# jinli99/iShapEditing

Measured on AMD Instinct MI355X. Metric: end-to-end drag-edit wall-clock (s) per shape, lower is better.
Workload: dtype f16; 1 GPU; C3 chair drag-edit: 3 handle->target pairs, 40 guided iterations (UNet fwd + drag gradient + UNet input-grad bwd + DDPM update) + 256^3 occupancy decode; unet=421M params, 1x96x128x128 latent, fp16 torso, r1=12, scale=1200

## Files before the change

### include/ishap.h

```cpp
#ifndef ISHAP_H
#define ISHAP_H
#ifdef __cplusplus
extern "C" {
#endif

const char* ishap_last_error(void);
int ishap_device_status(void);
int ishap_rendezvous_would_grant(const void* owner, void* stream);
int ishap_version(void);

typedef struct ishap_unet ishap_unet;

typedef struct {
  int image_size;
  int in_channels;
  int model_channels;
  int out_channels;
  int num_res_blocks;
  int n_mult;
  int channel_mult[8];
  int n_att;
  int attention_ds[8];
  int num_head_channels;
  int max_batch;
} ishap_unet_config;

int ishap_unet_create(const ishap_unet_config* cfg, int device, ishap_unet** out);
void ishap_unet_destroy(ishap_unet* u);

int ishap_unet_num_params(const ishap_unet* u);
int ishap_unet_param_info(const ishap_unet* u, int index, char* name, int name_cap, int* ndim, long long* shape);
int ishap_unet_load_param(ishap_unet* u, const char* name, const float* data, long long numel, void* stream);
int ishap_unet_params_loaded(const ishap_unet* u);

int ishap_unet_forward(ishap_unet* u, const float* x, const float* timesteps, int N, int feat_layer,
                       float* out, void* inter_feat, int keep_for_backward, void* stream);
int ishap_unet_tap_shape(const ishap_unet* u, int feat_layer, int* channels, int* size);
const void* ishap_unet_tap_ptr(const ishap_unet* u);
int ishap_unet_join_tail(ishap_unet* u, void* stream);
int ishap_unet_run_tail(ishap_unet* u);
int ishap_unet_marks(ishap_unet* u, int* tags, float* ms, int cap, float* tail_begin_ms, float* tail_end_ms);
int ishap_unet_copy_tap(const ishap_unet* u, void* dst, void* stream);
int ishap_unet_block_output(const ishap_unet* u, int group, int index, int* channels, int* size, void* dst_nchw_f16,
                            void* stream);
int ishap_unet_prepare_timesteps(ishap_unet* u, const float* timesteps, int n, void* stream);
long long ishap_unet_workspace_bytes(const ishap_unet* u);

int ishap_unet_snapshot_save(ishap_unet* u, void* stream);
int ishap_unet_snapshot_restore(ishap_unet* u, void* stream);
int ishap_unet_snapshot_drop(ishap_unet* u);
long long ishap_unet_snapshot_bytes(const ishap_unet* u);

int ishap_unet_backward_input(ishap_unet* u, const void* cot_nhwc, const float* scale2, float* dx, void* stream);
int ishap_unet_backward_from_output(ishap_unet* u, const void* cot_out, int cot_is_f16, const float* scale2, float* dx,
                                    void* stream);

long long ishap_group_norm32_scratch_bytes(int N, int HW, int C);
int ishap_group_norm32(const void* x_nhwc_f16, const float* gamma, const float* beta, int N, int H, int W, int C, int silu,
                       int route, void* y_nhwc_f16, float* stats, void* scratch, void* stream);
int ishap_group_norm32_backward(const void* g_nhwc_f16, const void* x_nhwc_f16, const float* stats, const float* gamma,
                                const float* beta, int N, int H, int W, int C, int silu, int route, void* dx_nhwc_f16,
                                void* scratch, void* stream);
int ishap_group_norm32_plan(int N, int H, int W, int C, int backward, int pending, int film, int act, int pool, int gmode, int route,
                            int* route_out, int* parts, int* vec, int* threads, int* grid_x, int* grid_y, int* lds_bytes,
                            int* xcd, char* kernel, int kernel_cap);

typedef struct {
  int backward, N, H, W, C, route, film, act;
  int pool, split;
  int gmode, sums_ready;
  int csplit, emb_ld;
  const float *gamma, *beta, *emb;
  void* scratch;
  const void *x, *x2;
  void *xcopy, *out, *xpool;
  float* stats_out;
  const long long *sums, *sums2;
  const void* g;
  const float* stats;
  const void *add, *add2;
  void *dx, *dx2;
  long long* csums;
  const float* ws;
  int nslab, ldr, res_ups, reserved_;
  long long zstride;
  const float *bias, *bias2;
  const void* res;
  void* ya;
} ishap_group_norm_desc;
int ishap_group_norm32_run(const ishap_group_norm_desc* d, int launch, void* stream, int* route_out, int* parts_out, char* kernel,
                           int kernel_cap);

typedef struct {
  float min_log;
  float max_log;
  float sqrt_recip;
  float sqrt_recipm1;
  float coef1, coef2;
  float nonzero;
  int clip_denoised;
  int mode;
  float ddim_a;
  float ddim_b;
  float ddim_sigma;
  int rng;
  unsigned long long rng_seed, rng_offset;
  float* noise_out;
} ishap_step_coefs;
int ishap_ddpm_step(const float* x, const float* model_out, const float* noise, const float* variance_in,
                    const ishap_step_coefs* k, int N, int C, int HW,
                    float* sample, float* pred_xstart, float* variance, float* mean, void* stream);
int ishap_ddpm_step_guided(const float* x, const float* model_out, const float* noise, const float* variance_in,
                           const ishap_step_coefs* k, int N, int C, int HW, const float* grad, float scale,
                           const float* grad_mul_dev, float* guided, float* sample, float* variance, void* stream);
int ishap_ddpm_step_guided_scales(const float* x, const float* model_out, const float* noise, const float* variance_in,
                                  const ishap_step_coefs* k, int N, int C, int HW, const float* grad, const float* scales,
                                  const float* grad_mul_dev, float* guided, float* sample, float* variance, void* stream);
int ishap_guided_update(const float* sample, const float* variance, const float* grad, float scale,
                        const float* grad_mul_dev, long long numel, float* out, void* stream);
int ishap_axpby(const float* x, const float* y, float a, float b, long long numel, float* out, void* stream);

typedef struct {
  int W;
  int ld;
  int Cc;
  const int* chmap;
  const float* sources;
  const float* targets;
// ... 194 lines not shown
```

### ishapediting_amd/_lib.py

```python
from __future__ import annotations

import ctypes as C
import os

HERE = os.path.dirname(os.path.abspath(__file__))
LIB_PATH = os.path.join(HERE, "libishap_hip.so")

c_float_p = C.POINTER(C.c_float)
c_void_p = C.c_void_p


class UNetConfigC(C.Structure):
    _fields_ = [("image_size", C.c_int), ("in_channels", C.c_int), ("model_channels", C.c_int),
                ("out_channels", C.c_int), ("num_res_blocks", C.c_int), ("n_mult", C.c_int),
                ("channel_mult", C.c_int * 8), ("n_att", C.c_int), ("attention_ds", C.c_int * 8),
                ("num_head_channels", C.c_int), ("max_batch", C.c_int)]


class StepCoefs(C.Structure):
    _fields_ = [("min_log", C.c_float), ("max_log", C.c_float), ("sqrt_recip", C.c_float),
                ("sqrt_recipm1", C.c_float), ("coef1", C.c_float), ("coef2", C.c_float),
                ("nonzero", C.c_float), ("clip_denoised", C.c_int), ("mode", C.c_int),
                ("ddim_a", C.c_float), ("ddim_b", C.c_float), ("ddim_sigma", C.c_float),
                ("rng", C.c_int), ("rng_seed", C.c_ulonglong), ("rng_offset", C.c_ulonglong), ("noise_out", c_void_p)]
# ... 9 lines not shown
    _fields_ = [("E", C.c_int), ("W", C.c_int), ("ld", C.c_int), ("Cc", C.c_int), ("chmap", c_void_p), ("sources", c_void_p),
                ("targets", c_void_p), ("handle_offsets", C.POINTER(C.c_int)), ("r", C.c_int), ("voxel", C.c_float),
                ("cof", C.POINTER(C.c_float)), ("l1", C.c_int), ("orig_stride", C.c_longlong), ("scratch", c_void_p),
                ("scratch_bytes", C.c_longlong)]


class IgemmBufC(C.Structure):
    _fields_ = [("ptr", c_void_p), ("bytes", C.c_longlong)]


class IgemmDescC(C.Structure):
    _fields_ = ([(f, C.c_int) for f in ("M", "N", "Cin", "taps", "K2", "H", "W", "ldx", "ldx2", "ldw", "ldo", "ldr", "ups",
                                        "res_ups", "out_mode", "pending", "chunk_tiles")] +
                [(f, IgemmBufC) for f in ("X", "X2", "Wt", "out", "bias", "bias2", "res", "ws", "stat_out", "gb_x", "gb_stats",
                                          "gb_gamma", "gb_beta", "gb_emb", "gb_csums")] +
                [("gb_emb_ld", C.c_int), ("gb_film", C.c_int), ("gb_act", C.c_int)])


class AttnDescC(C.Structure):
    _fields_ = ([(f, C.c_int) for f in ("pass_", "N", "T", "C", "heads", "d", "xcd_map")] +
                [(f, IgemmBufC) for f in ("qkv", "out", "lse", "dout", "dqkv")])


class Attn8DescC(C.Structure):
    _fields_ = ([(f, C.c_int) for f in ("N", "C", "heads")] +
                [(f, IgemmBufC) for f in ("xn", "wqkv", "bqkv", "wproj", "qkv", "aout", "lse", "slices", "flags")])


class GroupNormDescC(C.Structure):
    _fields_ = ([(f, C.c_int) for f in ("backward", "N", "H", "W", "C", "route", "film", "act", "pool", "split", "gmode",
                                        "sums_ready", "csplit", "emb_ld")] +
                [(f, c_void_p) for f in ("gamma", "beta", "emb", "scratch", "x", "x2", "xcopy", "out", "xpool", "stats_out", "sums",
                                         "sums2", "g", "stats", "add", "add2", "dx", "dx2", "csums", "ws")] +
                [(f, C.c_int) for f in ("nslab", "ldr", "res_ups", "reserved_")] + [("zstride", C.c_longlong)] +
                [(f, c_void_p) for f in ("bias", "bias2", "res", "ya")])


class DecoderWeightsC(C.Structure):
    _fields_ = [("B", c_void_p), ("W1", c_void_p), ("b1", c_void_p), ("W2", c_void_p), ("b2", c_void_p),
                ("w3", c_void_p), ("b3", c_void_p)]


class CameraC(C.Structure):
    _fields_ = [("eye", C.c_float * 3), ("centre", C.c_float * 3), ("up", C.c_float * 3), ("fov_y_deg", C.c_float),
                ("near", C.c_float), ("far", C.c_float)]


SYMBOLS = {
    "ishap_last_error": (C.c_char_p, []),
    "ishap_version": (C.c_int, []),
    "ishap_device_status": (C.c_int, []),
    "ishap_rendezvous_would_grant": (C.c_int, [C.c_void_p, C.c_void_p]),
    "ishap_group_norm32_scratch_bytes": (C.c_longlong, [C.c_int, C.c_int, C.c_int]),
    "ishap_group_norm32": (C.c_int, [c_void_p, c_void_p, c_void_p, C.c_int, C.c_int, C.c_int, C.c_int, C.c_int, C.c_int,
                                     c_void_p, c_void_p, c_void_p, c_void_p]),
    "ishap_group_norm32_backward": (C.c_int, [c_void_p, c_void_p, c_void_p, c_void_p, c_void_p, C.c_int, C.c_int, C.c_int,
                                              C.c_int, C.c_int, C.c_int, c_void_p, c_void_p, c_void_p]),
    "ishap_group_norm32_plan": (C.c_int, [C.c_int] * 11 + [C.POINTER(C.c_int)] * 8 + [C.c_char_p, C.c_int]),
    "ishap_group_norm32_run": (C.c_int, [C.POINTER(GroupNormDescC), C.c_int, c_void_p, C.POINTER(C.c_int), C.POINTER(C.c_int),
                                         C.c_char_p, C.c_int]),
    "ishap_unet_create": (C.c_int, [C.POINTER(UNetConfigC), C.c_int, C.POINTER(c_void_p)]),
    "ishap_unet_destroy": (None, [c_void_p]),
    "ishap_unet_num_params": (C.c_int, [c_void_p]),
    "ishap_unet_param_info": (C.c_int, [c_void_p, C.c_int, C.c_char_p, C.c_int, C.POINTER(C.c_int),
                                        C.POINTER(C.c_longlong)]),
    "ishap_unet_load_param": (C.c_int, [c_void_p, C.c_char_p, c_void_p, C.c_longlong, c_void_p]),
    "ishap_unet_params_loaded": (C.c_int, [c_void_p]),
    "ishap_unet_forward": (C.c_int, [c_void_p, c_void_p, c_float_p, C.c_int, C.c_int, c_void_p, c_void_p, C.c_int,
                                     c_void_p]),
    "ishap_unet_tap_shape": (C.c_int, [c_void_p, C.c_int, C.POINTER(C.c_int), C.POINTER(C.c_int)]),
    "ishap_unet_tap_ptr": (c_void_p, [c_void_p]),
    "ishap_unet_copy_tap": (C.c_int, [c_void_p, c_void_p, c_void_p]),
    "ishap_unet_block_output": (C.c_int, [c_void_p, C.c_int, C.c_int, C.POINTER(C.c_int), C.POINTER(C.c_int), c_void_p,
                                          c_void_p]),
    "ishap_unet_workspace_bytes": (C.c_longlong, [c_void_p]),
    "ishap_unet_join_tail": (C.c_int, [c_void_p, c_void_p]),
    "ishap_unet_run_tail": (C.c_int, [c_void_p]),
    "ishap_unet_snapshot_save": (C.c_int, [c_void_p, c_void_p]),
    "ishap_unet_snapshot_restore": (C.c_int, [c_void_p, c_void_p]),
    "ishap_unet_snapshot_drop": (C.c_int, [c_void_p]),
    "ishap_unet_snapshot_bytes": (C.c_longlong, [c_void_p]),
    "ishap_unet_marks": (C.c_int, [c_void_p, c_void_p, c_void_p, C.c_int, c_void_p, c_void_p]),
    "ishap_unet_prepare_timesteps": (C.c_int, [c_void_p, c_void_p, C.c_int, c_void_p]),
    "ishap_unet_backward_input": (C.c_int, [c_void_p, c_void_p, c_void_p, c_void_p, c_void_p]),
    "ishap_unet_backward_from_output": (C.c_int, [c_void_p, c_void_p, C.c_int, c_void_p, c_void_p, c_void_p]),
    "ishap_triplane_points_loss_grad": (C.c_int, [c_void_p, C.c_int, C.POINTER(DecoderWeightsC), c_void_p, c_void_p, c_void_p,
                                                  c_void_p, C.c_longlong, c_void_p, c_void_p, c_void_p, c_void_p]),
    "ishap_x0_grad_to_cotangent": (C.c_int, [c_void_p, c_void_p, c_void_p, c_void_p, C.c_float, C.c_float, C.c_int, C.c_int,
                                             c_void_p, c_void_p, c_void_p]),
    "ishap_ddpm_step": (C.c_int, [c_void_p, c_void_p, c_void_p, c_void_p, C.POINTER(StepCoefs), C.c_int, C.c_int,
                                  C.c_int, c_void_p, c_void_p, c_void_p, c_void_p, c_void_p]),
    "ishap_ddpm_step_guided": (C.c_int, [c_void_p, c_void_p, c_void_p, c_void_p, C.POINTER(StepCoefs), C.c_int, C.c_int, C.c_int,
                                         c_void_p, C.c_float, c_void_p, c_void_p, c_void_p, c_void_p, c_void_p]),
    "ishap_ddpm_step_guided_scales": (C.c_int, [c_void_p, c_void_p, c_void_p, c_void_p, C.POINTER(StepCoefs), C.c_int, C.c_int,
                                                C.c_int, c_void_p, c_void_p, c_void_p, c_void_p, c_void_p, c_void_p, c_void_p]),
    "ishap_guided_update": (C.c_int, [c_void_p, c_void_p, c_void_p, C.c_float, c_void_p, C.c_longlong, c_void_p,
                                      c_void_p]),
    "ishap_axpby": (C.c_int, [c_void_p, c_void_p, C.c_float, C.c_float, C.c_longlong, c_void_p, c_void_p]),
    "ishap_drag_setup": (C.c_int, [C.POINTER(DragArgsC), c_void_p]),
    "ishap_drag_loss_grad": (C.c_int, [C.POINTER(DragArgsC), c_void_p, c_void_p, c_void_p, c_void_p, c_void_p]),
    "ishap_drag_loss_cotangent": (C.c_int, [C.POINTER(DragArgsC), c_void_p, c_void_p, c_void_p, c_void_p, c_void_p, c_void_p,
                                            c_void_p, c_void_p]),
    "ishap_drag_batch_scratch_bytes": (C.c_longlong, [C.c_int, C.c_int, C.c_int]),
    "ishap_drag_batch_setup": (C.c_int, [C.POINTER(DragBatchArgsC), c_void_p]),
    "ishap_drag_batch_loss_grad": (C.c_int, [C.POINTER(DragBatchArgsC), c_void_p, c_void_p, c_void_p, c_void_p, c_void_p]),
    "ishap_drag_batch_loss_cotangent": (C.c_int, [C.POINTER(DragBatchArgsC), c_void_p, c_void_p, c_void_p, c_void_p, c_void_p,
                                                  c_void_p, c_void_p, c_void_p]),
    "ishap_grad_to_scaled_f16": (C.c_int, [c_void_p, c_void_p, c_void_p, c_void_p, C.c_longlong, c_void_p]),
    "ishap_planes_prepare": (C.c_int, [c_void_p, c_void_p, c_void_p, C.c_int, c_void_p, c_void_p]),
    "ishap_triplane_fit_loss_grad": (C.c_int, [c_void_p, C.c_int, C.POINTER(DecoderWeightsC), c_void_p, c_void_p, c_void_p,
                                               C.c_longlong, c_void_p, c_void_p, C.c_longlong, C.c_float, c_void_p, c_void_p,
                                               c_void_p]),
    "ishap_triplane_reg_adam_step": (C.c_int, [c_void_p, c_void_p, c_void_p, c_void_p, c_void_p, C.c_int, c_void_p, C.c_double,
                                               C.c_double, C.c_double, C.c_double, C.c_float, C.c_float, c_void_p, c_void_p,
                                               c_void_p]),
    "ishap_triplane_reg_values": (C.c_int, [c_void_p, C.c_int, c_void_p, c_void_p, c_void_p]),
    "ishap_triplane_decode_points": (C.c_int, [c_void_p, C.c_int, C.POINTER(DecoderWeightsC), c_void_p, C.c_longlong,
                                               c_void_p, c_void_p]),
    "ishap_surface_scratch_bytes": (C.c_longlong, [C.c_int]),
    "ishap_surface_count": (C.c_int, [c_void_p, C.c_int, C.c_float, C.c_int, c_void_p, c_void_p, c_void_p]),
    "ishap_surface_emit": (C.c_int, [c_void_p, C.c_int, C.c_float, C.c_int, c_void_p, c_void_p, c_void_p, c_void_p]),
    "ishap_mesh_smooth_scratch_bytes": (C.c_longlong, [C.c_longlong, C.c_longlong]),
    "ishap_mesh_smooth": (C.c_int, [c_void_p, C.c_longlong, c_void_p, C.c_longlong, C.c_int, C.c_float, c_void_p, C.c_longlong, c_void_p]),
    "ishap_chamfer": (C.c_int, [c_void_p, C.c_longlong, c_void_p, C.c_longlong, c_void_p, c_void_p, c_void_p]),
    "ishap_mesh_tri_areas": (C.c_int, [c_void_p, c_void_p, C.c_longlong, c_void_p, c_void_p]),
    "ishap_mesh_points_on_tris": (C.c_int, [c_void_p, c_void_p, c_void_p, c_void_p, C.c_longlong, c_void_p, c_void_p]),
    "ishap_mesh_occupancy": (C.c_int, [c_void_p, c_void_p, C.c_longlong, c_void_p, C.c_longlong, c_void_p, c_void_p]),
    "ishap_mesh_distance_scratch_bytes": (C.c_longlong, [C.c_longlong]),
    "ishap_mesh_distance": (C.c_int, [c_void_p, c_void_p, C.c_longlong, c_void_p, C.c_longlong, C.c_int, c_void_p, c_void_p,
                                      c_void_p, C.c_longlong, c_void_p]),
    "ishap_mesh_distance_scratch_bytes_sdf": (C.c_longlong, [C.c_longlong, C.c_longlong, C.c_int]),
    "ishap_hausdorff": (C.c_int, [c_void_p, C.c_longlong, c_void_p, C.c_longlong, c_void_p, c_void_p, c_void_p]),
    "ishap_winding_scratch_bytes": (C.c_longlong, [C.c_longlong, C.c_longlong]),
    "ishap_mesh_winding": (C.c_int, [c_void_p, c_void_p, C.c_longlong, c_void_p, C.c_longlong, c_void_p, c_void_p, C.c_longlong,
                                     c_void_p]),
    "ishap_cloud_winding": (C.c_int, [c_void_p, c_void_p, c_void_p, C.c_longlong, c_void_p, C.c_longlong, c_void_p, c_void_p,
                                      C.c_longlong, c_void_p]),
    "ishap_cloud_areas": (C.c_int, [c_void_p, C.c_longlong, C.c_int, c_void_p, c_void_p]),
    "ishap_cloud_knn": (C.c_int, [c_void_p, C.c_longlong, C.c_int, c_void_p, c_void_p, c_void_p]),
    "ishap_cloud_normals": (C.c_int, [c_void_p, C.c_longlong, c_void_p, C.c_int, c_void_p, c_void_p, c_void_p]),
    "ishap_cloud_orient_scratch_bytes": (C.c_longlong, [C.c_longlong]),
    "ishap_cloud_orient": (C.c_int, [c_void_p, c_void_p, c_void_p, C.c_longlong, C.c_int, c_void_p, C.c_longlong,
                                     C.POINTER(C.c_int), c_void_p]),
    "ishap_volume_label": (C.c_int, [c_void_p, C.c_int, C.c_int, C.c_int, C.c_float, C.c_int, C.c_int, c_void_p, c_void_p]),
    "ishap_volume_components_scratch_bytes": (C.c_longlong, [C.c_longlong]),
    "ishap_volume_components_count": (C.c_int, [c_void_p, C.c_int, C.c_int, C.c_int, c_void_p, c_void_p, c_void_p]),
    "ishap_volume_components_emit": (C.c_int, [c_void_p, C.c_int, C.c_int, C.c_int, c_void_p, c_void_p, c_void_p]),
    "ishap_volume_flip": (C.c_int, [c_void_p, c_void_p, c_void_p, C.c_int, C.c_int, C.c_int, C.c_float, c_void_p, C.c_longlong,
                                    c_void_p, c_void_p]),
    "ishap_group_field_stats": (C.c_int, [c_void_p, c_void_p, C.c_int, C.c_longlong, C.c_int, c_void_p, c_void_p]),
    "ishap_arap_scratch_bytes": (C.c_longlong, [C.c_longlong, C.c_longlong, C.c_longlong]),
    "ishap_arap": (C.c_int, [c_void_p, C.c_longlong, c_void_p, C.c_longlong, c_void_p, c_void_p, C.c_longlong, C.c_int, C.c_double,
                             C.c_longlong, c_void_p, c_void_p, c_void_p, c_void_p, C.c_longlong, c_void_p]),
    "ishap_nearest_vertices": (C.c_int, [c_void_p, C.c_longlong, c_void_p, C.c_longlong, c_void_p, c_void_p]),
    "ishap_render_scratch_bytes": (C.c_longlong, [C.c_longlong, C.c_longlong, C.c_int, C.c_int]),
    "ishap_render_mesh": (C.c_int, [c_void_p, C.c_longlong, c_void_p, C.c_longlong, c_void_p, c_void_p, c_void_p, C.c_int,
                                    C.POINTER(CameraC), C.c_int, C.c_int, c_void_p, C.c_longlong, c_void_p, c_void_p, c_void_p,
                                    c_void_p]),
    "ishap_unproject": (C.c_int, [C.POINTER(CameraC), C.c_int, C.c_int, c_void_p, C.c_longlong, c_void_p, c_void_p]),
    "ishap_profile_begin": (C.c_int, []),
    "ishap_profile_end": (C.c_int, [C.POINTER(C.c_double), C.c_int]),
    "ishap_profile_shapes": (C.c_int, [C.c_char_p, C.c_int]),
    "ishap_igemm_plan": (C.c_int, [C.c_int] * 10 + [C.POINTER(C.c_int), C.POINTER(C.c_int), C.c_char_p, C.c_int]),
    "ishap_igemm_run": (C.c_int, [C.POINTER(IgemmDescC), C.c_int, c_void_p, C.POINTER(C.c_int), C.c_char_p, C.c_int]),
    "ishap_igemm_reduce": (C.c_int, [C.POINTER(IgemmDescC), C.c_int, C.c_int, c_void_p]),
    "ishap_attention_run": (C.c_int, [C.POINTER(AttnDescC), C.c_int, c_void_p, C.c_char_p, C.c_int]),
    "ishap_attention8_run": (C.c_int, [C.POINTER(Attn8DescC), C.c_int, C.c_int, c_void_p, C.POINTER(C.c_int)]),
    "ishap_triplane_decode_grid": (C.c_int, [c_void_p, C.c_int, C.POINTER(DecoderWeightsC), c_void_p, C.c_int,
                                             c_void_p, c_void_p]),
}

_lib = None


def lib():
    global _lib
    if _lib is None:
        if not os.path.exists(LIB_PATH):
            raise RuntimeError(
                f"{LIB_PATH} is missing: the HIP extension is required (no CPU fallback exists). "
                "Build it with `python -m ishapediting_amd.build`.")
        import torch
        tlib = os.path.join(os.path.dirname(torch.__file__), "lib", "libamdhip64.so")
        if os.path.exists(tlib):
            C.CDLL(tlib, mode=C.RTLD_GLOBAL)
        l = C.CDLL(LIB_PATH)
        for name, (res, args) in SYMBOLS.items():
            fn = getattr(l, name)
            fn.restype = res
            fn.argtypes = args
        if l.ishap_version() < 16:
            raise RuntimeError(f"{LIB_PATH} is an older build (ABI {l.ishap_version()} < 16): rebuild with `python -m ishapediting_amd.build`")
        _lib = l
    return _lib


def check(rc: int):
    if rc != 0:
        msg = lib().ishap_last_error()
        raise RuntimeError(f"libishap_hip: {msg.decode() if msg else 'error'} (code {rc})")


def ptr(t):
    return None if t is None else t.data_ptr()


def stream_ptr(device=None):
    import torch
    return torch.cuda.current_stream(device).cuda_stream
```

### ishapediting_amd/csrc/misc.hip

```cpp
#include "misc.h"

__global__ __launch_bounds__(256) void nchw_to_nhwc_kernel(const float* __restrict__ src, half_t* __restrict__ dst,
                                                           int C, int HW, int Cpad, int ytiles, uint4* __restrict__ zero, long long zero_n16) {
  __shared__ float tile[32][33];
  const int n = blockIdx.z;
  if ((int)blockIdx.y >= ytiles) {
    const long long nb = (long long)gridDim.x * (gridDim.y - ytiles) * gridDim.z;
    const long long b = blockIdx.x + (long long)gridDim.x * ((blockIdx.y - ytiles) + (long long)(gridDim.y - ytiles) * blockIdx.z);
    for (long long i = b * 256 + threadIdx.x; i < zero_n16; i += nb * 256) zero[i] = make_uint4(0u, 0u, 0u, 0u);
    return;
  }
  const int p0 = blockIdx.x * 32, c0 = blockIdx.y * 32;
  const int tx = threadIdx.x & 31, ty = threadIdx.x >> 5;
  for (int j = ty; j < 32; j += 8) {
    int c = c0 + j, p = p0 + tx;
    tile[j][tx] = (c < C && p < HW) ? src[((long long)n * C + c) * HW + p] : 0.f;
  }
  __syncthreads();
  for (int j = ty; j < 32; j += 8) {
    int p = p0 + j, c = c0 + tx;
    if (p < HW && c < Cpad) dst[((long long)n * HW + p) * Cpad + c] = (half_t)tile[tx][j];
  }
}
int nchw_f32_to_nhwc_f16(const float* src, half_t* dst, int N, int C, int HW, int Cpad, hipStream_t s, void* zero, size_t zero_bytes) {
// ... 43 lines not shown
  const int tx = threadIdx.x & 31, ty = threadIdx.x >> 5;
  for (int j = ty; j < 32; j += 8) {
    int c = c0 + j, p = p0 + tx;
    tile[j][tx] = (c < C && p < HW) ? (float)src[((long long)n * C + c) * HW + p] * mul : 0.f;
  }
  __syncthreads();
  for (int j = ty; j < 32; j += 8) {
    int p = p0 + j, c = c0 + tx;
    if (p < HW && c < ld) dst[((long long)n * HW + p) * ld + c] = (half_t)tile[tx][j];
  }
}
int nchw_to_nhwc_f16_scaled(const void* src, int src_f32, half_t* dst, int N, int C, int HW, int ld, float mul,
                            hipStream_t s) {
  dim3 g(ceil_div(HW, 32), ceil_div(ld, 32), N);
  if (src_f32) hipLaunchKernelGGL(nchw_any_to_nhwc_kernel<float>, g, dim3(256), 0, s, (const float*)src, dst, C, HW, ld, mul);
  else hipLaunchKernelGGL(nchw_any_to_nhwc_kernel<half_t>, g, dim3(256), 0, s, (const half_t*)src, dst, C, HW, ld, mul);
  ISHAP_CHECK_HIP(hipGetLastError());
  return 0;
}

__global__ void concat2_kernel(const half_t* __restrict__ a, const half_t* __restrict__ b, half_t* __restrict__ o,
                               long long M, int Ca, int Cb, const long long* __restrict__ sa,
                               const long long* __restrict__ sb, long long* __restrict__ so, int N) {
  if (so && blockIdx.x == 0) {
    const int Cc = Ca + Cb;
    for (int i = threadIdx.x; i < N * Cc * 2; i += blockDim.x) {
      const int k = i & 1, c = (i >> 1) % Cc, n = (i >> 1) / Cc;
      so[i] = c < Ca ? sa[(n * Ca + c) * 2 + k] : sb[(n * Cb + (c - Ca)) * 2 + k];
    }
  }
  const int CV = (Ca + Cb) >> 3, CVa = Ca >> 3;
  const long long total = M * CV;
  for (long long i = (long long)blockIdx.x * blockDim.x + threadIdx.x; i < total; i += (long long)gridDim.x * blockDim.x) {
    long long m = i / CV;
    int cv = (int)(i % CV);
    half8 v = cv < CVa ? *reinterpret_cast<const half8*>(a + m * Ca + cv * 8)
                       : *reinterpret_cast<const half8*>(b + m * Cb + (cv - CVa) * 8);
    *reinterpret_cast<half8*>(o + m * (Ca + Cb) + cv * 8) = v;
  }
}
int concat2(const half_t* a, const half_t* b, half_t* o, long long M, int Ca, int Cb, hipStream_t s, const long long* sa,
            const long long* sb, long long* so, int N) {
  long long total = M * ((Ca + Cb) / 8);
  int blocks = (int)std::min<long long>((total + 255) / 256, 4096);
  hipLaunchKernelGGL(concat2_kernel, dim3(blocks), dim3(256), 0, s, a, b, o, M, Ca, Cb, sa, sb, so, N);
  ISHAP_CHECK_HIP(hipGetLastError());
  return 0;
}

__global__ void add_kernel(const half_t* __restrict__ a, const half_t* __restrict__ b, half_t* __restrict__ o, long long nvec) {
  for (long long i = (long long)blockIdx.x * blockDim.x + threadIdx.x; i < nvec; i += (long long)gridDim.x * blockDim.x) {
    half8 x = reinterpret_cast<const half8*>(a)[i], y = reinterpret_cast<const half8*>(b)[i], r;
#pragma unroll
    for (int k = 0; k < 8; ++k) r[k] = (half_t)((float)x[k] + (float)y[k]);
    reinterpret_cast<half8*>(o)[i] = r;
  }
}
int add_f16(const half_t* a, const half_t* b, half_t* o, long long n, hipStream_t s) {
  long long nvec = n / 8;
  int blocks = (int)std::min<long long>((nvec + 255) / 256, 4096);
  hipLaunchKernelGGL(add_kernel, dim3(blocks), dim3(256), 0, s, a, b, o, nvec);
  ISHAP_CHECK_HIP(hipGetLastError());
  return 0;
}


__global__ void timestep_embedding_kernel(TsArg t, float* __restrict__ out, int dim) {
  const int n = blockIdx.x;
  const int half = dim / 2;
  for (int j = threadIdx.x; j < half; j += blockDim.x) {
    float f = expf(-logf(10000.f) * (float)j / (float)half);
    float a = t.t[n] * f;
    out[n * dim + j] = cosf(a);
    out[n * dim + half + j] = sinf(a);
  }
  if ((dim & 1) && threadIdx.x == 0) out[n * dim + dim - 1] = 0.f;
}
int timestep_embedding(const TsArg& t, float* out, int N, int dim, hipStream_t s) {
  hipLaunchKernelGGL(timestep_embedding_kernel, dim3(N), dim3(128), 0, s, t, out, dim);
  ISHAP_CHECK_HIP(hipGetLastError());
  return 0;
}

__global__ __launch_bounds__(256) void gemv_kernel(const float* __restrict__ W, const float* __restrict__ b,
                                                   const float* __restrict__ in, float* __restrict__ out, int rows, int K,
                                                   int N, int silu_in) {
  const int row = blockIdx.x * 4 + (threadIdx.x >> 6);
  const int lane = threadIdx.x & 63;
  if (row >= rows) return;
  const float* w = W + (long long)row * K;
  for (int n = 0; n < N; ++n) {
    float acc = 0.f;
    for (int k = lane * 4; k < K; k += 256) {
      f32x4 wv = *reinterpret_cast<const f32x4*>(w + k);
      f32x4 xv = *reinterpret_cast<const f32x4*>(in + (long long)n * K + k);
#pragma unroll
      for (int i = 0; i < 4; ++i) {
        float x = xv[i];
        if (silu_in) x = x / (1.f + __expf(-x));
        acc += wv[i] * x;
      }
    }
    for (int o = 32; o > 0; o >>= 1) acc += __shfl_xor(acc, o);
    if (lane == 0) out[(long long)n * rows + row] = acc + b[row];
  }
}
int gemv_f32(const float* W, const float* b, const float* in, float* out, int rows, int K, int N, int silu_in,
             hipStream_t s) {
  ISHAP_REQUIRE(K % 4 == 0, "gemv K % 4");
  hipLaunchKernelGGL(gemv_kernel, dim3(ceil_div(rows, 4)), dim3(256), 0, s, W, b, in, out, rows, K, N, silu_in);
  ISHAP_CHECK_HIP(hipGetLastError());
  return 0;
}

__global__ void pack_conv_kernel(const float* __restrict__ w, half_t* __restrict__ dst, int O, int I, int taps,
                                 int rows_pad, int cpad, int transpose_flip, int dst_ld, int col_off) {
  const long long total = (long long)rows_pad * taps * cpad;
  for (long long i = (long long)blockIdx.x * blockDim.x + threadIdx.x; i < total; i += (long long)gridDim.x * blockDim.x) {
    int c = (int)(i % cpad);
    int tap = (int)((i / cpad) % taps);
    int r = (int)(i / ((long long)cpad * taps));
    float v = 0.f;
    if (!transpose_flip) {
      if (r < O && c < I) v = w[((long long)r * I + c) * taps + tap];
    } else {
      if (r < I && c < O) v = w[((long long)c * I + r) * taps + (taps - 1 - tap)];
    }
    dst[(long long)r * dst_ld + col_off + tap * cpad + c] = (half_t)v;
  }
}
int pack_conv_weight(const float* w, half_t* dst, int O, int I, int taps, int rows_pad, int cpad, int transpose_flip,
                     hipStream_t s, int dst_ld, int col_off) {
  long long total = (long long)rows_pad * taps * cpad;
  int blocks = (int)std::min<long long>((total + 255) / 256, 8192);
  hipLaunchKernelGGL(pack_conv_kernel, dim3(blocks), dim3(256), 0, s, w, dst, O, I, taps, rows_pad, cpad, transpose_flip,
                     dst_ld ? dst_ld : taps * cpad, col_off);
  ISHAP_CHECK_HIP(hipGetLastError());
  return 0;
}

__global__ void pack_conv_split_kernel(const float* __restrict__ w, half_t* __restrict__ dst, int O, int I, int taps,
                                       int rows_pad) {
  const int cpad = 3 * I;
  const long long total = (long long)rows_pad * taps * cpad;
  for (long long i = (long long)blockIdx.x * blockDim.x + threadIdx.x; i < total; i += (long long)gridDim.x * blockDim.x) {
    int c3 = (int)(i % cpad);
    int tap = (int)((i / cpad) % taps);
    int r = (int)(i / ((long long)cpad * taps));
    int part = c3 / I, c = c3 % I;
    float v = 0.f;
    if (r < O) {
      float f = w[((long long)r * I + c) * taps + tap];
      half_t hi = (half_t)f;
      v = (part < 2) ? (float)hi : (f - (float)hi);
    }
    dst[i] = (half_t)v;
  }
}
int pack_conv_weight_split(const float* w, half_t* dst, int O, int I, int taps, int rows_pad, hipStream_t s) {
  long long total = (long long)rows_pad * taps * 3 * I;
  int blocks = (int)std::min<long long>((total + 255) / 256, 8192);
  hipLaunchKernelGGL(pack_conv_split_kernel, dim3(blocks), dim3(256), 0, s, w, dst, O, I, taps, rows_pad);
  ISHAP_CHECK_HIP(hipGetLastError());
  return 0;
}

__global__ void round_f16_kernel(const float* __restrict__ src, float* __restrict__ dst, long long n) {
  for (long long i = (long long)blockIdx.x * blockDim.x + threadIdx.x; i < n; i += (long long)gridDim.x * blockDim.x)
    dst[i] = (float)(half_t)src[i];
}
int round_through_f16(const float* src, float* dst, long long n, hipStream_t s) {
  int blocks = (int)std::min<long long>((n + 255) / 256, 4096);
  hipLaunchKernelGGL(round_f16_kernel, dim3(blocks), dim3(256), 0, s, src, dst, n);
  ISHAP_CHECK_HIP(hipGetLastError());
  return 0;
}

__global__ __launch_bounds__(256) void nhwc_to_nchw_scaled_kernel(const half_t* __restrict__ src, float* __restrict__ dst,
                                                                  int C, int HW, int ld, const float* __restrict__ mul_dev) {
  __shared__ float tile[32][33];
  const float mul = mul_dev ? *mul_dev : 1.f;
  const int n = blockIdx.z;
  const int p0 = blockIdx.x * 32, c0 = blockIdx.y * 32;
  const int tx = threadIdx.x & 31, ty = threadIdx.x >> 5;
  for (int j = ty; j < 32; j += 8) {
    int p = p0 + j, c = c0 + tx;
    tile[j][tx] = (c < C && p < HW) ? (float)src[((long long)n * HW + p) * ld + c] * mul : 0.f;
  }
  __syncthreads();
  for (int j = ty; j < 32; j += 8) {
    int c = c0 + j, p = p0 + tx;
    if (c < C && p < HW) dst[((long long)n * C + c) * HW + p] = tile[tx][j];
  }
// ... 9 lines not shown
```

### ishapediting_amd/csrc/unet.h

```cpp
#pragma once
#include <map>
#include <string>
#include <vector>

#include "../../include/ishap.h"
#include "common.h"

struct Tensor {
  half_t* p = nullptr;
  int N = 0, H = 0, W = 0, C = 0;
  long long* sums = nullptr;
  const half_t* cat_a = nullptr; const half_t* cat_b = nullptr; const long long* cat_sa = nullptr; const long long* cat_sb = nullptr;
  int cat_ca = 0;
  SlabSrc pend, cat_pend;
  long long rows() const { return (long long)N * H * W; }
  long long numel() const { return rows() * C; }
};

struct Arena {
  char* base = nullptr;
  size_t cap = 0, off = 0, high = 0;
  bool dry = false;
  void reset() { off = 0; }
  void* alloc(size_t bytes) {
// ... 33 lines not shown
  Tensor x, qkv, a;
  float* stats = nullptr;
  float* lse = nullptr;
};

struct ResL {
  std::string path;
  int cin = 0, cout = 0;
  bool up = false, down = false;
  NormW n1, n2;
  ConvW c1, c2, skip;
  bool has_skip = false;
  int emb_off = 0;
  ResSaved sv;
};
struct AttnL {
  std::string path;
  int C = 0, heads = 0;
  NormW n;
  ConvW qkv, proj;
  AttnSaved sv;
};
struct LayerRef { int kind; int idx; };
struct BlockL {
  std::string name;
  std::vector<LayerRef> layers;
  int cin = 0, cout = 0, res_in = 0, res_out = 0, skip_ch = 0;
  Tensor out;
  Tensor cat;
};

struct ParamSlot {
  std::string name;
  int ndim = 0;
  long long shape[4] = {0, 0, 0, 0};
  int kind = 0;
  ConvW* conv = nullptr;
  float* dst = nullptr;
  long long dst_off = 0;
  bool loaded = false;
  long long numel() const {
    long long n = 1;
    for (int i = 0; i < ndim; ++i) n *= shape[i];
    return n;
  }
};

struct UnetSnapshot {
  bool valid = false;
  bool partial = false;
  char* arena = nullptr;      size_t arena_cap = 0, arena_bytes = 0;
  long long* stat = nullptr;  size_t stat_cap = 0, stat_count = 0;
  float* film = nullptr;      size_t film_cap = 0, film_floats = 0;
  int film_ld = 0;
  size_t fwd_mark = 0, stat_fwd_mark = 0;
  int last_N = 0, last_feat = -1;
  Tensor tap, x0, h_final;
  float* head_stats = nullptr;
  std::vector<ResSaved> res;
  std::vector<AttnSaved> attn;
  std::vector<Tensor> outs, cats;
  size_t bytes() const { return arena_cap + stat_cap * sizeof(long long) + film_cap * sizeof(float); }
};

struct ishap_unet {
  ishap_unet_config cfg;
  int device = 0;
  int ted = 0;
  int in_pad = 0;
  ConvW stem, head;
  NormW head_norm;
  std::vector<ResL> res;
  std::vector<AttnL> attn;
  std::vector<BlockL> in_blocks, out_blocks;
  BlockL mid;
  int final_ch = 0;
  float *te_w0 = nullptr, *te_b0 = nullptr, *te_w2 = nullptr, *te_b2 = nullptr;
  float *emb_w = nullptr, *emb_b = nullptr;
  int film_rows = 0;
  float *d_temb = nullptr, *d_e1 = nullptr, *d_emb = nullptr, *d_film = nullptr;
  float* film_cache = nullptr;
  size_t film_cache_rows = 0;
  std::vector<float> film_cache_ts;
  float *pc_temb = nullptr, *pc_e1 = nullptr, *pc_emb = nullptr;
  const float* film_cur = nullptr;
  int film_cur_ld = 0;
  std::vector<ParamSlot> params;
  std::map<std::string, int> param_index;
  int n_loaded = 0;
  Arena arena;
  float* ws = nullptr;          size_t ws_floats = 0;
  float* gn_partial = nullptr;  size_t gn_partial_floats = 0;
  int last_N = 0, last_feat = -1;
  bool have_saved = false;
  Tensor tap;
  Tensor x0, h_final;
  float* head_stats = nullptr;
  long long* stat_base = nullptr;
  size_t stat_cap = 0, stat_off = 0, stat_high = 0, stat_fwd_mark = 0;
  int bwd_since_fwd = 0;
  size_t fwd_mark = 0;
  hipStream_t side = nullptr;
  hipEvent_t ev_fork = nullptr, ev_tail = nullptr, ev_mid = nullptr;
  bool marks_on = false;
  std::vector<hipEvent_t> marks;
  std::vector<int> mark_tags;
  int marks_n = 0;
  hipEvent_t mark_tail_begin = nullptr, mark_tail_end = nullptr;
  bool mark_tail_set = false;
  bool tail_pending = false;
  struct TailState { size_t split; Tensor h; std::vector<Tensor> hs; int N; float* out; size_t arena_off, stat_off; bool keep; };
  TailState tail{};
  bool tail_deferred = false, mid_recorded = false;
  float* ws_side = nullptr;
  float* gn_partial_side = nullptr;
  float* attn_D = nullptr;
  size_t attn_D_floats = 0;
  bool last_overlap = false;
  UnetSnapshot snap;
  bool restored_partial = false;
};

struct Exec {
  ishap_unet* u;
  hipStream_t s;
  bool dry;
  bool keep = false;
  float* ws = nullptr;
  float* gn_partial = nullptr;
  int chunk_tiles = 0;
  bool tenant = true;
};
template <typename T>
static inline int aalloc_checked(Exec& e, size_t count, T** out) {
  *out = (T*)e.u->arena.alloc(count * sizeof(T));
  ISHAP_REQUIRE(*out != nullptr, "activation arena exhausted (shape beyond what ishap_unet_create sized for)");
  return 0;
}
#define ISHAP_ALLOC(ptr, e, count) ISHAP_TRY(aalloc_checked((e), (size_t)(count), &(ptr)))
#define ISHAP_SALLOC(ptr, e, count)                                                                   \
  do {                                                                                                \
    (ptr) = salloc((e), (size_t)(count));                                                             \
    ISHAP_REQUIRE((ptr) != nullptr, "GroupNorm statistics arena exhausted");                          \
  } while (0)
int conv_op(Exec& e, const ConvLaunch& c);
ConvLaunch conv_launch(const Tensor& x, const ConvW& w, const Tensor& y);
int unet_join_tail(ishap_unet* u, hipStream_t s);
bool ishap_profile_recording();
bool exec_is_solo(const Exec& e);
int slab_materialize(Exec& e, Tensor& t);
long long* salloc(Exec& e, size_t count);
int gn_stats_op(Exec& e, const Tensor& x, float* stats);

int unet_build(ishap_unet* u);
int unet_forward_impl(ishap_unet* u, const float* x, const float* ts, int N, int feat_layer, float* out,
                      void* inter_feat, int keep, hipStream_t s, bool dry);
int unet_backward_impl(ishap_unet* u, const half_t* cot_tap, const void* cot_out, int cot_out_f16, const float* scale2,
                       float* dx, hipStream_t s, bool dry);
```

### ishapediting_amd/csrc/unet.hip

```cpp
#include "unet.h"

#include <cstring>

#include "attention.h"
#include "decode.h"
#include "misc.h"
#include "norm.h"

static int round_up(int a, int b) { return (a + b - 1) / b * b; }

static void init_conv(ConvW& c, const std::string& path, int cin, int cout, int taps) {
  c.path = path; c.cin = cin; c.cout = cout; c.taps = taps;
  c.kpad = round_up(cin, 32);
  c.cout_pad = round_up(cout, 32);
}

int unet_build(ishap_unet* u) {
  const ishap_unet_config& cfg = u->cfg;
  const int mc = cfg.model_channels;
  u->ted = mc * 4;
  u->in_pad = cfg.in_channels >= 64 ? round_up(cfg.in_channels, 64) : round_up(cfg.in_channels, 32);
  auto has_att = [&](int ds) {
    for (int i = 0; i < cfg.n_att; ++i) if (cfg.attention_ds[i] == ds) return true;
    return false;
// ... 561 lines not shown
      for (size_t k = 0; k < u->film_cache_ts.size() && !prepared; ++k)
        if (u->film_cache_ts[k] == ts[0]) {
          u->film_cur = u->film_cache + k * (size_t)u->film_rows;
          u->film_cur_ld = 0;
          prepared = true;
        }
  }
  if (!dry && !prepared) {
    TsArg ta;
    for (int i = 0; i < 16; ++i) ta.t[i] = i < N ? ts[i] : 0.f;
    ISHAP_TRY(timestep_embedding(ta, u->d_temb, N, cfg.model_channels, s));
    ISHAP_TRY(gemv_f32(u->te_w0, u->te_b0, u->d_temb, u->d_e1, u->ted, cfg.model_channels, N, 0, s));
    ISHAP_TRY(gemv_f32(u->te_w2, u->te_b2, u->d_e1, u->d_emb, u->ted, u->ted, N, 1, s));
    ISHAP_TRY(gemv_f32(u->emb_w, u->emb_b, u->d_emb, u->d_film, u->film_rows, u->ted, N, 1, s));
  }
  Tensor h{nullptr, N, S, S, u->in_pad};
  ISHAP_ALLOC(h.p, e, h.numel());
  if (!dry) ISHAP_TRY(nchw_f32_to_nhwc_f16(x, h.p, N, cfg.in_channels, HW, u->in_pad, s, zero_in_convert ? u->stat_base : nullptr,
                                           zero_in_convert ? u->stat_cap * sizeof(long long) : 0));
  u->x0 = h;
  std::vector<Tensor> hs;
  for (auto& b : u->in_blocks) {
    Tensor y;
    ISHAP_TRY(block_forward(e, b, h, y));
    h = y;
    hs.push_back(h);
    hs.back().pend = SlabSrc{};
  }
  {
    Tensor y;
    ISHAP_TRY(block_forward(e, u->mid, h, y));
    h = y;
  }
  u->tap = Tensor{};
  const size_t n_out = u->out_blocks.size();
  const size_t split = overlap ? (size_t)feat_layer + 1 : n_out;
  ISHAP_TRY(out_blocks_range(e, u, 0, split, h, hs, feat_layer));
  if (overlap) {
    ISHAP_TRY(slab_materialize(e, h));
    u->tap = h;
    ISHAP_CHECK_HIP(hipEventRecord(u->ev_fork, s));
    u->tail = ishap_unet::TailState{split, h, hs, N, out, u->arena.off, u->stat_off, (keep & 1) != 0};
    Exec plan = e;
    plan.dry = true;
    Tensor hp = h;
    std::vector<Tensor> hsp = hs;
    ISHAP_TRY(out_blocks_range(plan, u, split, n_out, hp, hsp, feat_layer));
    ISHAP_TRY(forward_head(plan, u, hp, N, out));
    u->tail_deferred = true;
    u->mid_recorded = false;
  } else {
    ISHAP_TRY(forward_head(e, u, h, N, out));
  }
  if (feat_layer >= 0 && inter_feat && !dry)
    ISHAP_TRY(nhwc_f16_to_nchw(u->tap.p, inter_feat, 0, N, u->tap.C, u->tap.H * u->tap.W, u->tap.C, s));
  u->last_N = N;
  u->last_feat = feat_layer;
  u->last_overlap = overlap;
  u->have_saved = (keep & 1) != 0 && !dry;
  u->fwd_mark = u->arena.off;
  u->stat_fwd_mark = u->stat_off;
  u->bwd_since_fwd = 0;
  return 0;
}

static void snap_blocks(ishap_unet* u, std::vector<BlockL*>& v) {
  for (auto& b : u->in_blocks) v.push_back(&b);
  v.push_back(&u->mid);
  for (auto& b : u->out_blocks) v.push_back(&b);
}
template <typename T>
static int snap_reserve(T** buf, size_t* cap, size_t need) {
  if (need <= *cap) return 0;
  if (*buf) ISHAP_CHECK_HIP(hipFree(*buf));
  *buf = nullptr;
  *cap = 0;
  ISHAP_CHECK_HIP(hipMalloc((void**)buf, need * sizeof(T)));
  *cap = need;
  return 0;
}

extern "C" {

int ishap_version(void) { return 16; }

int ishap_unet_create(const ishap_unet_config* cfg, int device, ishap_unet** out) {
  ISHAP_REQUIRE(cfg && out, "null argument");
  ISHAP_REQUIRE(cfg->n_mult >= 1 && cfg->n_mult <= 8 && cfg->n_att <= 8, "config arrays");
  ISHAP_REQUIRE(cfg->model_channels % 32 == 0, "model_channels must be a multiple of 32 (GroupNorm32)");
  ISHAP_REQUIRE(cfg->num_head_channels > 0 && cfg->num_head_channels % 32 == 0, "num_head_channels % 32");
  ISHAP_REQUIRE(cfg->out_channels % 4 == 0, "out_channels % 4");
  ISHAP_REQUIRE(cfg->max_batch >= 1 && cfg->max_batch <= 16, "max_batch in [1,16]");
  int minres = cfg->image_size >> (cfg->n_mult - 1);
  ISHAP_REQUIRE(minres * minres >= 64 && (cfg->image_size & (cfg->image_size - 1)) == 0,
                "image_size: power of two with at least 8x8 at the deepest level");
  ISHAP_CHECK_HIP(hipSetDevice(device));
  ishap_unet* u = new ishap_unet();
  u->cfg = *cfg;
  u->marks_on = ishap_switch("ISHAP_BWD_MARKS", 0) != 0;
  u->device = device;
  int r = unet_build(u);
  if (r) { delete u; return r; }
  u->arena.dry = true;
  std::vector<float> ts(cfg->max_batch, 0.f);
  for (int nb = 1; nb <= cfg->max_batch && !r; ++nb) {
    r = unet_forward_impl(u, nullptr, ts.data(), nb, (int)u->out_blocks.size() - 1, nullptr, nullptr, 1, 0, true);
    if (!r) r = unet_backward_impl(u, nullptr, (const void*)0x1000, 0, nullptr, nullptr, 0, true);
  }
  if (r) { delete u; return r; }
  u->arena.dry = false;
  u->arena.cap = align_up(u->arena.high + (1 << 20), 1 << 20);
  ISHAP_CHECK_HIP(hipMalloc((void**)&u->arena.base, u->arena.cap));
  if (u->ws_floats) ISHAP_CHECK_HIP(hipMalloc((void**)&u->ws, u->ws_floats * sizeof(float)));
  ISHAP_CHECK_HIP(hipMalloc((void**)&u->gn_partial, std::max<size_t>(u->gn_partial_floats, 64) * sizeof(float)));
  u->stat_cap = (u->stat_high + 1023) / 1024 * 1024;
  ISHAP_CHECK_HIP(hipMalloc((void**)&u->stat_base, std::max<size_t>(u->stat_cap, 1024) * sizeof(long long)));
  if (u->attn_D_floats) ISHAP_CHECK_HIP(hipMalloc((void**)&u->attn_D, u->attn_D_floats * sizeof(float)));
  u->have_saved = false;
  *out = u;
  return 0;
}

void ishap_unet_destroy(ishap_unet* u) {
  if (!u) return;
  auto fr = [](void* p) { if (p) (void)hipFree(p); };
  auto frc = [&](ConvW& c) { fr(c.w); fr(c.wT); fr(c.bias); if (c.cat && c.cat_off == 0) fr(c.cat); };
  frc(u->stem); frc(u->head);
  fr(u->head_norm.gamma); fr(u->head_norm.beta);
  for (auto& r : u->res) {
    frc(r.c1); frc(r.c2); if (r.has_skip) frc(r.skip);
    fr(r.n1.gamma); fr(r.n1.beta); fr(r.n2.gamma); fr(r.n2.beta);
  }
  for (auto& a : u->attn) { frc(a.qkv); frc(a.proj); fr(a.n.gamma); fr(a.n.beta); }
  fr(u->te_w0); fr(u->te_b0); fr(u->te_w2); fr(u->te_b2); fr(u->emb_w); fr(u->emb_b);
  fr(u->d_temb); fr(u->d_e1); fr(u->d_emb); fr(u->d_film);
  fr(u->film_cache); fr(u->pc_temb); fr(u->pc_e1); fr(u->pc_emb);
  fr(u->ws_side); fr(u->gn_partial_side);
  fr(u->snap.arena); fr(u->snap.stat); fr(u->snap.film);
  if (u->side) (void)hipStreamDestroy(u->side);
  if (u->ev_fork) (void)hipEventDestroy(u->ev_fork);
  if (u->ev_tail) (void)hipEventDestroy(u->ev_tail);
  if (u->ev_mid) (void)hipEventDestroy(u->ev_mid);
  for (hipEvent_t ev : u->marks) (void)hipEventDestroy(ev);
  if (u->mark_tail_begin) (void)hipEventDestroy(u->mark_tail_begin);
  if (u->mark_tail_end) (void)hipEventDestroy(u->mark_tail_end);
  fr(u->arena.base); fr(u->ws); fr(u->gn_partial); fr(u->attn_D); fr(u->stat_base);
  delete u;
}

int ishap_unet_num_params(const ishap_unet* u) { return u ? (int)u->params.size() : 0; }

int ishap_unet_param_info(const ishap_unet* u, int index, char* name, int name_cap, int* ndim, long long* shape) {
  ISHAP_REQUIRE(u && index >= 0 && index < (int)u->params.size(), "param index");
  const ParamSlot& p = u->params[index];
  if (name && name_cap > 0) {
    std::strncpy(name, p.name.c_str(), name_cap - 1);
    name[name_cap - 1] = 0;
  }
  if (ndim) *ndim = p.ndim;
  if (shape) for (int i = 0; i < 4; ++i) shape[i] = p.shape[i];
  return 0;
}

int ishap_unet_load_param(ishap_unet* u, const char* name, const float* data, long long numel, void* stream) {
  ISHAP_REQUIRE(u && name && data, "null argument");
  auto it = u->param_index.find(name);
  ISHAP_REQUIRE(it != u->param_index.end(), std::string("unexpected key in state_dict: ") + name);
  ParamSlot& p = u->params[it->second];
  ISHAP_REQUIRE(p.numel() == numel, std::string("size mismatch for ") + name);
  ISHAP_CHECK_HIP(hipSetDevice(u->device));
  ISHAP_TRY(load_param(u, p, data, (hipStream_t)stream));
  if (!p.loaded) { p.loaded = true; u->n_loaded++; }
  u->film_cache_ts.clear();
  u->snap.valid = false;
  return 0;
}

int ishap_unet_prepare_timesteps(ishap_unet* u, const float* ts, int n, void* stream) {
  ISHAP_REQUIRE(u && (ts || n == 0) && n >= 0 && n <= 4096, "prepare_timesteps arguments");
  ISHAP_CHECK_HIP(hipSetDevice(u->device));
  hipStream_t s = (hipStream_t)stream;
  u->film_cache_ts.clear();
  if (u->film_cur != u->d_film) { u->have_saved = false; u->film_cur = u->d_film; u->film_cur_ld = u->film_rows; }
  if (n == 0) return 0;
  ISHAP_REQUIRE(u->n_loaded == (int)u->params.size(), "prepare_timesteps before all parameters are loaded");
  const int mc = u->cfg.model_channels;
  if ((size_t)n > u->film_cache_rows) {
    if (u->film_cache) ISHAP_CHECK_HIP(hipFree(u->film_cache));
    u->film_cache = nullptr;
    u->film_cache_rows = 0;
    ISHAP_CHECK_HIP(hipMalloc((void**)&u->film_cache, (size_t)n * u->film_rows * sizeof(float)));
    u->film_cache_rows = (size_t)n;
  }
  if (!u->pc_temb) {
    ISHAP_CHECK_HIP(hipMalloc((void**)&u->pc_temb, (size_t)16 * mc * sizeof(float)));
    ISHAP_CHECK_HIP(hipMalloc((void**)&u->pc_e1, (size_t)16 * u->ted * sizeof(float)));
    ISHAP_CHECK_HIP(hipMalloc((void**)&u->pc_emb, (size_t)16 * u->ted * sizeof(float)));
  }
  for (int c0 = 0; c0 < n; c0 += 16) {
    const int m = std::min(16, n - c0);
    TsArg ta;
    for (int i = 0; i < 16; ++i) ta.t[i] = i < m ? ts[c0 + i] : 0.f;
    ISHAP_TRY(timestep_embedding(ta, u->pc_temb, m, mc, s));
    ISHAP_TRY(gemv_f32(u->te_w0, u->te_b0, u->pc_temb, u->pc_e1, u->ted, mc, m, 0, s));
    ISHAP_TRY(gemv_f32(u->te_w2, u->te_b2, u->pc_e1, u->pc_emb, u->ted, u->ted, m, 1, s));
    ISHAP_TRY(gemv_f32(u->emb_w, u->emb_b, u->pc_emb, u->film_cache + (size_t)c0 * u->film_rows, u->film_rows, u->ted, m, 1, s));
  }
  u->film_cache_ts.assign(ts, ts + n);
  return 0;
}

int ishap_unet_params_loaded(const ishap_unet* u) { return u ? u->n_loaded : 0; }

int ishap_unet_join_tail(ishap_unet* u, void* stream) {
  ISHAP_REQUIRE(u, "null argument");
  ISHAP_CHECK_HIP(hipSetDevice(u->device));
  return unet_join_tail(u, (hipStream_t)stream);
}

int ishap_unet_run_tail(ishap_unet* u) {
  ISHAP_REQUIRE(u, "null argument");
  ISHAP_CHECK_HIP(hipSetDevice(u->device));
  return unet_run_tail(u);
}

int ishap_unet_forward(ishap_unet* u, const float* x, const float* timesteps, int N, int feat_layer, float* out,
                       void* inter_feat, int keep_for_backward, void* stream) {
  ISHAP_REQUIRE(u && x && timesteps && out, "null argument");
  ISHAP_REQUIRE(u->n_loaded == (int)u->params.size(), "missing keys: not every state_dict tensor has been loaded");
  ISHAP_TRY(ishap_check_status());
  ISHAP_CHECK_HIP(hipSetDevice(u->device));
  return unet_forward_impl(u, x, timesteps, N, feat_layer, out, inter_feat, keep_for_backward, (hipStream_t)stream, false);
}

int ishap_unet_tap_shape(const ishap_unet* u, int feat_layer, int* channels, int* size) {
  ISHAP_REQUIRE(u && feat_layer >= 0 && feat_layer < (int)u->out_blocks.size(), "feat_layer out of range");
  if (channels) *channels = u->out_blocks[feat_layer].cout;
  if (size) *size = u->out_blocks[feat_layer].res_out;
  return 0;
}

const void* ishap_unet_tap_ptr(const ishap_unet* u) { return u ? u->tap.p : nullptr; }

long long ishap_unet_workspace_bytes(const ishap_unet* u) {
  if (!u) return 0;
  return (long long)(u->arena.cap + u->ws_floats * sizeof(float) + u->gn_partial_floats * sizeof(float) +
                     u->stat_cap * sizeof(long long) + u->attn_D_floats * sizeof(float) + u->snap.bytes());
}

int ishap_unet_block_output(const ishap_unet* u, int group, int index, int* channels, int* size, void* dst_nchw_f16,
                            void* stream) {
  ISHAP_REQUIRE(u && group >= 0 && group <= 2, "group: 0 input_blocks, 1 middle_block, 2 output_blocks");
  const BlockL* b = nullptr;
  if (group == 0) { ISHAP_REQUIRE(index >= 0 && index < (int)u->in_blocks.size(), "input block index"); b = &u->in_blocks[index]; }
  else if (group == 1) b = &u->mid;
  else { ISHAP_REQUIRE(index >= 0 && index < (int)u->out_blocks.size(), "output block index"); b = &u->out_blocks[index]; }
  if (channels) *channels = b->cout;
  if (size) *size = b->res_out;
  if (!dst_nchw_f16) return 0;
  ISHAP_REQUIRE(u->have_saved && b->out.p, "block outputs stay resident only after a forward with keep_for_backward=1");
  ISHAP_REQUIRE(!(u->restored_partial && group == 2 && index > u->last_feat), "the restored snapshot holds the network up to the tap only");
  ISHAP_TRY(ishap_check_status());
  ISHAP_CHECK_HIP(hipSetDevice(u->device));
  ISHAP_TRY(unet_join_tail(const_cast<ishap_unet*>(u), (hipStream_t)stream));
  return nhwc_f16_to_nchw(b->out.p, dst_nchw_f16, 0, b->out.N, b->out.C, b->out.H * b->out.W, b->out.C, (hipStream_t)stream);
}

int ishap_unet_copy_tap(const ishap_unet* u, void* dst, void* stream) {
  ISHAP_REQUIRE(u && dst && u->tap.p, "no resident tap (run a forward with feat_layer >= 0 first)");
  ISHAP_CHECK_HIP(hipMemcpyAsync(dst, u->tap.p, (size_t)u->tap.numel() * sizeof(half_t), hipMemcpyDeviceToDevice,
                                 (hipStream_t)stream));
  return 0;
}

int ishap_unet_snapshot_save(ishap_unet* u, void* stream) {
  ISHAP_REQUIRE(u, "null argument");
  ISHAP_REQUIRE(u->have_saved, "a snapshot needs a preceding forward with keep_for_backward=1");
  if (ishap_profile_recording()) return 1;
  if (u->snap.film && u->film_cur == u->snap.film) {
    ISHAP_REQUIRE(u->snap.valid, "the kept state came from a snapshot that is no longer valid");
    return 0;
  }
  ISHAP_TRY(ishap_check_status());
  ISHAP_CHECK_HIP(hipSetDevice(u->device));
  hipStream_t s = (hipStream_t)stream;
  ISHAP_TRY(unet_join_tail(u, s));
  UnetSnapshot& sn = u->snap;
  sn.valid = false;
  sn.partial = u->last_overlap;
  sn.arena_bytes = sn.partial ? u->tail.arena_off : u->fwd_mark;
  sn.stat_count = sn.partial ? u->tail.stat_off : u->stat_fwd_mark;
  sn.film_ld = u->film_cur_ld;
  sn.film_floats = (size_t)u->film_rows * (sn.film_ld ? (size_t)u->last_N : 1);
// ... 72 lines not shown
```

Measured before the change: 0.1600 s/shape.

## Batch timestep GEMV over all timesteps with LDS-staged inputs and skip recomputing cached FiLM rows

Rewrites the FP32 GEMV used for timestep embedding and FiLM projection. It stages all N input vectors (with SiLU applied once) in LDS and accumulates every timestep per weight row in registers, so each weight row is read once instead of once per timestep. It also makes prepare_timesteps return early when every requested timestep is already in the FiLM cache, and adds a counter of computed rows. The cost is a 64 KB LDS limit on N*K and a new early-return path that must stay consistent with the cache-state resets that were skipped.

```diff
diff --git a/include/ishap.h b/include/ishap.h
--- a/include/ishap.h
+++ b/include/ishap.h
@@ -44,6 +44,7 @@
 int ishap_unet_block_output(const ishap_unet* u, int group, int index, int* channels, int* size, void* dst_nchw_f16,
                             void* stream);
 int ishap_unet_prepare_timesteps(ishap_unet* u, const float* timesteps, int n, void* stream);
+long long ishap_unet_film_rows_computed(const ishap_unet* u);
 long long ishap_unet_workspace_bytes(const ishap_unet* u);
 
 int ishap_unet_snapshot_save(ishap_unet* u, void* stream);
diff --git a/ishapediting_amd/_lib.py b/ishapediting_amd/_lib.py
--- a/ishapediting_amd/_lib.py
+++ b/ishapediting_amd/_lib.py
@@ -115,6 +115,7 @@
     "ishap_unet_snapshot_bytes": (C.c_longlong, [c_void_p]),
     "ishap_unet_marks": (C.c_int, [c_void_p, c_void_p, c_void_p, C.c_int, c_void_p, c_void_p]),
     "ishap_unet_prepare_timesteps": (C.c_int, [c_void_p, c_void_p, C.c_int, c_void_p]),
+    "ishap_unet_film_rows_computed": (C.c_longlong, [c_void_p]),
     "ishap_unet_backward_input": (C.c_int, [c_void_p, c_void_p, c_void_p, c_void_p, c_void_p]),
     "ishap_unet_backward_from_output": (C.c_int, [c_void_p, c_void_p, C.c_int, c_void_p, c_void_p, c_void_p]),
     "ishap_triplane_points_loss_grad": (C.c_int, [c_void_p, C.c_int, C.POINTER(DecoderWeightsC), c_void_p, c_void_p, c_void_p,
@@ -222,8 +223,8 @@
             fn = getattr(l, name)
             fn.restype = res
             fn.argtypes = args
-        if l.ishap_version() < 16:
-            raise RuntimeError(f"{LIB_PATH} is an older build (ABI {l.ishap_version()} < 16): rebuild with `python -m ishapediting_amd.build`")
+        if l.ishap_version() < 17:
+            raise RuntimeError(f"{LIB_PATH} is an older build (ABI {l.ishap_version()} < 17): rebuild with `python -m ishapediting_amd.build`")
         _lib = l
     return _lib
 
diff --git a/ishapediting_amd/csrc/misc.hip b/ishapediting_amd/csrc/misc.hip
--- a/ishapediting_amd/csrc/misc.hip
+++ b/ishapediting_amd/csrc/misc.hip
@@ -149,33 +149,68 @@
   return 0;
 }
 
-__global__ __launch_bounds__(256) void gemv_kernel(const float* __restrict__ W, const float* __restrict__ b,
-                                                   const float* __restrict__ in, float* __restrict__ out, int rows, int K,
-                                                   int N, int silu_in) {
-  const int row = blockIdx.x * 4 + (threadIdx.x >> 6);
+constexpr int GEMV_THREADS = 512, GEMV_WAVES = GEMV_THREADS / 64, GEMV_MAX_N = 16, GEMV_LDS_BYTES = 64 * 1024;
+template <int NT>
+__global__ __launch_bounds__(GEMV_THREADS) void gemv_kernel(const float* __restrict__ W, const float* __restrict__ b,
+                                                            const float* __restrict__ in, float* __restrict__ out, int rows,
+                                                            int K, int silu_in) {
+  extern __shared__ __attribute__((aligned(16))) float gemv_x[];
+  for (int i = threadIdx.x * 4; i < NT * K; i += GEMV_THREADS * 4) {
+    f32x4 xv = *reinterpret_cast<const f32x4*>(in + i);
+    if (silu_in) {
+#pragma unroll
+      for (int j = 0; j < 4; ++j) {
+        float x = xv[j];
+        xv[j] = x / (1.f + __expf(-x));
+      }
+    }
+    *reinterpret_cast<f32x4*>(gemv_x + i) = xv;
+  }
+  __syncthreads();
   const int lane = threadIdx.x & 63;
-  if (row >= rows) return;
-  const float* w = W + (long long)row * K;
-  for (int n = 0; n < N; ++n) {
-    float acc = 0.f;
+  for (int row = blockIdx.x * GEMV_WAVES + (threadIdx.x >> 6); row < rows; row += gridDim.x * GEMV_WAVES) {
+    const float* w = W + (long long)row * K;
+    float acc[NT];
+#pragma unroll
+    for (int n = 0; n < NT; ++n) acc[n] = 0.f;
+#pragma unroll 4
     for (int k = lane * 4; k < K; k += 256) {
       f32x4 wv = *reinterpret_cast<const f32x4*>(w + k);
-      f32x4 xv = *reinterpret_cast<const f32x4*>(in + (long long)n * K + k);
-#pragma unroll
-      for (int i = 0; i < 4; ++i) {
-        float x = xv[i];
-        if (silu_in) x = x / (1.f + __expf(-x));
-        acc += wv[i] * x;
+#pragma unroll
+      for (int n = 0; n < NT; ++n) {
+        f32x4 xv = *reinterpret_cast<const f32x4*>(gemv_x + n * K + k);
+#pragma unroll
+        for (int i = 0; i < 4; ++i) acc[n] = __builtin_fmaf(wv[i], xv[i], acc[n]);
       }
     }
-    for (int o = 32; o > 0; o >>= 1) acc += __shfl_xor(acc, o);
-    if (lane == 0) out[(long long)n * rows + row] = acc + b[row];
-  }
+    const float bias = b[row];
+#pragma unroll
+    for (int n = 0; n < NT; ++n) {
+      float a = acc[n];
+      for (int o = 32; o > 0; o >>= 1) a += __shfl_xor(a, o);
+      if (lane == 0) out[(long long)n * rows + row] = a + bias;
+    }
+  }
+}
+template <int NT>
+static void gemv_launch(const float* W, const float* b, const float* in, float* out, int rows, int K, int silu_in,
+                        hipStream_t s) {
+  const int blocks = std::min(ceil_div(rows, GEMV_WAVES), 512);
+  hipLaunchKernelGGL(gemv_kernel<NT>, dim3(blocks), dim3(GEMV_THREADS), (size_t)NT * K * sizeof(float), s, W, b, in, out, rows,
+                     K, silu_in);
 }
 int gemv_f32(const float* W, const float* b, const float* in, float* out, int rows, int K, int N, int silu_in,
              hipStream_t s) {
   ISHAP_REQUIRE(K % 4 == 0, "gemv K % 4");
-  hipLaunchKernelGGL(gemv_kernel, dim3(ceil_div(rows, 4)), dim3(256), 0, s, W, b, in, out, rows, K, N, silu_in);
+  ISHAP_REQUIRE(N >= 1 && N <= GEMV_MAX_N && (long long)N * K * (long long)sizeof(float) <= GEMV_LDS_BYTES,
+                "gemv: 1..16 timesteps, N * K floats within 64 KB of LDS");
+  switch (N) {
+#define ISHAP_GEMV_CASE(n) case n: gemv_launch<n>(W, b, in, out, rows, K, silu_in, s); break;
+    ISHAP_GEMV_CASE(1) ISHAP_GEMV_CASE(2) ISHAP_GEMV_CASE(3) ISHAP_GEMV_CASE(4) ISHAP_GEMV_CASE(5) ISHAP_GEMV_CASE(6)
+    ISHAP_GEMV_CASE(7) ISHAP_GEMV_CASE(8) ISHAP_GEMV_CASE(9) ISHAP_GEMV_CASE(10) ISHAP_GEMV_CASE(11) ISHAP_GEMV_CASE(12)
+    ISHAP_GEMV_CASE(13) ISHAP_GEMV_CASE(14) ISHAP_GEMV_CASE(15) ISHAP_GEMV_CASE(16)
+#undef ISHAP_GEMV_CASE
+  }
   ISHAP_CHECK_HIP(hipGetLastError());
   return 0;
 }
diff --git a/ishapediting_amd/csrc/unet.h b/ishapediting_amd/csrc/unet.h
--- a/ishapediting_amd/csrc/unet.h
+++ b/ishapediting_amd/csrc/unet.h
@@ -139,6 +139,7 @@
   float* film_cache = nullptr;
   size_t film_cache_rows = 0;
   std::vector<float> film_cache_ts;
+  long long film_rows_computed = 0;
   float *pc_temb = nullptr, *pc_e1 = nullptr, *pc_emb = nullptr;
   const float* film_cur = nullptr;
   int film_cur_ld = 0;
diff --git a/ishapediting_amd/csrc/unet.hip b/ishapediting_amd/csrc/unet.hip
--- a/ishapediting_amd/csrc/unet.hip
+++ b/ishapediting_amd/csrc/unet.hip
@@ -667,7 +667,7 @@
 
 extern "C" {
 
-int ishap_version(void) { return 16; }
+int ishap_version(void) { return 17; }
 
 int ishap_unet_create(const ishap_unet_config* cfg, int device, ishap_unet** out) {
   ISHAP_REQUIRE(cfg && out, "null argument");
@@ -765,6 +765,12 @@
   ISHAP_REQUIRE(u && (ts || n == 0) && n >= 0 && n <= 4096, "prepare_timesteps arguments");
   ISHAP_CHECK_HIP(hipSetDevice(u->device));
   hipStream_t s = (hipStream_t)stream;
+  if (n > 0 && !u->film_cache_ts.empty()) {
+    bool hit = true;
+    for (int i = 0; i < n && hit; ++i)
+      hit = std::find(u->film_cache_ts.begin(), u->film_cache_ts.end(), ts[i]) != u->film_cache_ts.end();
+    if (hit) return 0;
+  }
   u->film_cache_ts.clear();
   if (u->film_cur != u->d_film) { u->have_saved = false; u->film_cur = u->d_film; u->film_cur_ld = u->film_rows; }
   if (n == 0) return 0;
@@ -790,10 +796,13 @@
     ISHAP_TRY(gemv_f32(u->te_w0, u->te_b0, u->pc_temb, u->pc_e1, u->ted, mc, m, 0, s));
     ISHAP_TRY(gemv_f32(u->te_w2, u->te_b2, u->pc_e1, u->pc_emb, u->ted, u->ted, m, 1, s));
     ISHAP_TRY(gemv_f32(u->emb_w, u->emb_b, u->pc_emb, u->film_cache + (size_t)c0 * u->film_rows, u->film_rows, u->ted, m, 1, s));
+    u->film_rows_computed += m;
   }
   u->film_cache_ts.assign(ts, ts + n);
   return 0;
 }
+
+long long ishap_unet_film_rows_computed(const ishap_unet* u) { return u ? u->film_rows_computed : 0; }
 
 int ishap_unet_params_loaded(const ishap_unet* u) { return u ? u->n_loaded : 0; }
 
```

New measurement: 0.1588 s/shape, median of 6. About the same (-0.8%).
